# Priberam/Enhance-CB-Whisper

Measured on AMD Instinct MI355X. Metric: utterances/sec (30 s clips) + keywords/sec matched, Whisper-large-v3 LEF 10k kw, higher is better.
Workload: dtype bf16

## Files before the change

enhance-cb-whisper_amd/csrc/conv_igemm.hip:

```cpp
#include "cbw_common.h"
#include "cbw_kernels.h"
#include "conv_route.h"

#include <atomic>

thread_local const char* cbw_last_conv_kernel = "";

int cbw_num_cus() {
    static std::atomic<int> cache[16];
    int dev = 0, n = 0;
    (void)hipGetDevice(&dev);
    const bool slot = dev >= 0 && dev < 16;
    if (slot && (n = cache[dev].load(std::memory_order_relaxed)) > 0) return n;
    if (hipDeviceGetAttribute(&n, hipDeviceAttributeMultiprocessorCount, dev) != hipSuccess || n <= 0) n = 256;
    if (slot) cache[dev].store(n, std::memory_order_relaxed);
    return n;
}

namespace {

constexpr int BK = 64;
constexpr int EPI_LD = 68;
constexpr int EPI_BYTES = 4 * 64 * EPI_LD * 4;
template <int BM, int BN>
// ... 586 lines not shown
        const char* B = A + BIG_BM * 64;
        bf16x8 av[FM], bv[4];
#pragma unroll
        for (int j = 0; j < 4; ++j) {
            const int r = wn * 64 + j * 16 + fr;
            bv[j] = *(const bf16x8*)(B + r * 64 + ((fq ^ swz4(r)) * 16));
        }
#pragma unroll
        for (int i = 0; i < FH; ++i) {
            const int r = wm * (FM * 16) + i * 16 + fr;
            av[i] = *(const bf16x8*)(A + r * 64 + ((fq ^ swz4(r)) * 16));
        }
#pragma unroll
        for (int i = 0; i < FH; ++i) {
            __builtin_amdgcn_sched_barrier(0);
            __builtin_amdgcn_s_setprio(1);
#pragma unroll
            for (int j = 0; j < 4; ++j)
                acc[i][j] = __builtin_amdgcn_mfma_f32_16x16x32_bf16(bv[j], av[i], acc[i][j], 0, 0, 0);
            __builtin_amdgcn_s_setprio(0);
            __builtin_amdgcn_sched_barrier(0);
            const int r = wm * (FM * 16) + (i + FH) * 16 + fr;
            av[i + FH] = *(const bf16x8*)(A + r * 64 + ((fq ^ swz4(r)) * 16));
        }
        __builtin_amdgcn_sched_barrier(0);
        if (s + 3 < nsteps) issue_next();
        __builtin_amdgcn_sched_barrier(0);
        __builtin_amdgcn_s_setprio(1);
#pragma unroll
        for (int i = FH; i < FM; ++i)
#pragma unroll
            for (int j = 0; j < 4; ++j)
                acc[i][j] = __builtin_amdgcn_mfma_f32_16x16x32_bf16(bv[j], av[i], acc[i][j], 0, 0, 0);
        __builtin_amdgcn_s_setprio(0);
        asm volatile("" ::: "memory");
    }

    const bool relu = a.flags & CBW_EPI_RELU;
    const bool split3 = a.flags & CBW_EPI_SPLIT3;
#pragma unroll
    for (int j = 0; j < 4; ++j) {
        const int col = n0 + wn * 64 + j * 16 + fq * 4;
        const f32x4 bb = a.bias ? *(const f32x4*)(a.bias + col) : f32x4{0.f, 0.f, 0.f, 0.f};
#pragma unroll
        for (int i = 0; i < FM; ++i) {
            const int m = m0 + wm * (FM * 16) + i * 16 + fr;
            if (m >= a.M) continue;
            f32x4 v;
#pragma unroll
            for (int q = 0; q < 4; ++q) {
                v[q] = acc[i][j][q] + bb[q];
                if (relu) v[q] = fmaxf(v[q], 0.f);
            }
            bf16x4 o;
#pragma unroll
            for (int q = 0; q < 4; ++q) o[q] = f2bf(v[q]);
            bf16* yp = (bf16*)a.y + (int64_t)m * a.y_ld + col;
            *(bf16x4*)yp = o;
            if (split3) {
                bf16x4 lo;
#pragma unroll
                for (int q = 0; q < 4; ++q) lo[q] = f2bf(v[q] - bf2f(o[q]));
                *(bf16x4*)(yp + a.Cout) = lo;
                if (a.y32) *(f32x4*)(a.y32 + (int64_t)m * a.Cout + col) = v;
            }
        }
    }
}

template <int BN, int KH, int KW>
hipError_t launch_big(const ConvArgs& a, int nt, hipStream_t st) {
    constexpr int lds = BIG_NS * (BIG_BM + BN) * 64;
    hipLaunchKernelGGL((conv_igemm_big2<BN, KH, KW>), dim3(nt), dim3(512), lds, st, a);
    return hipGetLastError();
}

constexpr int P8_BM = 256, P8_BN = 256, P8_BK = 64;
CBW_DEV int p8_off(int r, int c) { return r * 128 + ((c ^ ((r >> 1) & 7)) << 4); }
template <int BN> struct P8Shape {
    static constexpr int BM = 65536 / BN;
    static constexpr int NA = BM / 128, NB = BN / 128;
    static constexpr int WCN = BN / 64;
    static constexpr int BUF = (BM + BN) * 128;
};
template <int N> CBW_DEV void vm_wait() {
    static_assert(N >= 0 && N <= 15, "vm_wait");
    asm volatile("s_waitcnt vmcnt(%0)" ::"n"(N) : "memory");
}

template <int KH, int KW, int BN = 256>
__global__ __launch_bounds__(512, 1) void conv_igemm_p8(ConvArgs a) {
    static_assert(KH * KW <= 32, "tap mask");
    using S = P8Shape<BN>;
    constexpr int BM = S::BM, NA = S::NA, NB = S::NB, WCN = S::WCN;
    extern __shared__ __attribute__((aligned(16))) char smem[];
    const int tid = threadIdx.x, lane = tid & 63, wid = tid >> 6;
    const int wr = (wid >> 2) * (4 / WCN) + (wid & 3) / WCN, wc = (wid & 3) % WCN;
    const int fr = lane & 15, fq = lane >> 4;
    const int nt_n = a.Cout / BN;
    const int nt_m = (a.M + BM - 1) / BM;
    const int bid = xcd_remap(blockIdx.x, nt_m * nt_n);
    const int tm = bid / nt_n, tn = bid % nt_n;
    const int m0 = tm * BM, n0 = tn * BN;
    const int cin2 = a.x2 ? a.Cin2 : 0;
    const int Ktot = KH * KW * a.Cin + cin2;
    const int csteps = a.Cin / P8_BK;
    const int nk1 = KH * KW * csteps;
    const int nk = nk1 + cin2 / P8_BK;
    const int HoWo = a.Ho * a.Wo;
    const int xld = a.x_ld ? a.x_ld : a.Cin;

    const int sub = lane >> 3, pch = lane & 7;
    const bf16* a_px[2][NA];
    const bf16* a2_px[2][NA];
    unsigned a_tm[2][NA];
    const bf16* wrow[2][NB];
    constexpr bool ROWS = KH * KW > 1;
    bool rowmap = false;
    int kh_lo = 0, kt_lo = 0, kt_hi = nk;
    if constexpr (ROWS) {
        rowmap = a.p8_g > 0;
        if (rowmap) {
            if (tid < BM) {
                int4 rec{-1, 0, 0, 0};
                if (m0 + tid < a.M) p8_row_pixel(m0 + tid, a.N, a.Ho, a.Wo, a.p8_g, rec.x, rec.y, rec.z, rec.w);
                ((int4*)smem)[tid] = rec;
            }
            __syncthreads();
            const int4 first = ((const int4*)smem)[0], last = ((const int4*)smem)[min(BM, a.M - m0) - 1];
            int kh_hi;
            p8_kh_range(__builtin_amdgcn_readfirstlane(first.y), __builtin_amdgcn_readfirstlane(last.y),
                        __builtin_amdgcn_readfirstlane(first.w) == __builtin_amdgcn_readfirstlane(last.w), a.H, a.sh,
                        a.ph, KH, kh_lo, kh_hi);
            kt_lo = kh_lo * KW * csteps;
            kt_hi = kh_hi * KW * csteps;
        }
    }
#pragma unroll
    for (int h = 0; h < 2; ++h)
#pragma unroll
        for (int g = 0; g < NA; ++g) {
            const int r = g * 128 + h * 64 + wid * 8 + sub;
            bool okm;
            int n, oh, ow;
            if (ROWS && rowmap) {
                const int4 rec = ((const int4*)smem)[r];
                okm = rec.x >= 0;
                n = okm ? rec.x : 0;
                oh = rec.y;
                ow = rec.z;
            } else {
                const int m = m0 + r;
                okm = m < a.M;
                const int mm = okm ? m : 0;
                n = mm / HoWo;
                const int rem = mm - n * HoWo;
                oh = rem / a.Wo;
                ow = rem - oh * a.Wo;
            }
            const int ih0 = oh * a.sh - a.ph, iw0 = ow * a.sw - a.pw;
            a2_px[h][g] = a.x2 ? (const bf16*)a.x2 + (((int64_t)n * a.H2 + oh * a.s2) * a.W2 + ow * a.s2) * cin2 +
                                     ((pch ^ ((r >> 1) & 7)) * 8)
                               : nullptr;
            unsigned tmask = 0;
#pragma unroll
            for (int kh = 0; kh < KH; ++kh)
#pragma unroll
                for (int kw = 0; kw < KW; ++kw) {
                    const int ih = ih0 + kh, iw = iw0 + kw;
                    if (okm && ih >= 0 && ih < a.H && iw >= 0 && iw < a.W) tmask |= 1u << (kh * KW + kw);
                }
            a_tm[h][g] = tmask;
            a_px[h][g] = (const bf16*)a.x + (int64_t)n * a.H * a.W * xld + ((int64_t)ih0 * a.W + iw0) * xld +
                         ((pch ^ ((r >> 1) & 7)) * 8);
        }
#pragma unroll
    for (int h = 0; h < 2; ++h)
#pragma unroll
        for (int g = 0; g < NB; ++g) {
            const int rb = h * (BN / 2) + g * 64 + wid * 8 + sub;
            const int rs = (rb & ~31) | (((rb & 15) >> 2) << 3) | (((rb >> 4) & 1) << 2) | (rb & 3);
            wrow[h][g] = (const bf16*)a.w + (int64_t)(n0 + rs) * Ktot + ((pch ^ ((rb >> 1) & 7)) * 8);
        }
    int nx_cs = 0, nx_tap = 0, nx_kh = 0, nx_kw = 0;
    if constexpr (ROWS) {
        nx_kh = kh_lo;
        nx_tap = nx_kh * KW;
        if (rowmap) __syncthreads();
    }
    int nx_off = nx_kh * a.W * xld + fold_c(0, a.xfold);
    auto advance = [&]() {
        if (++nx_cs == csteps) {
            nx_cs = 0;
            ++nx_tap;
            if (++nx_kw == KW) { nx_kw = 0; ++nx_kh; }
        }
        nx_off = (nx_kh * a.W + nx_kw) * xld + fold_c(nx_cs * P8_BK, a.xfold);
    };
    auto issue = [&](int kt, int which) {
        char* A = smem + (kt & 1) * S::BUF;
        if (which == 0 || which == 3) {
            const int h = which == 3;
            if (kt >= nk1) {
                const int c0 = (kt - nk1) * P8_BK;
#pragma unroll
                for (int g = 0; g < NA; ++g) {
                    const void* src = (a_tm[h][g] & 1u) ? (const void*)(a2_px[h][g] + c0) : a.zero;
                    __builtin_amdgcn_global_load_lds(src, (void*)(A + (g * 128 + h * 64 + wid * 8) * 128), 16, 0, 0);
                }
                return;
            }
            const int tap = nx_tap;
            const int toff = nx_off;
#pragma unroll
            for (int g = 0; g < NA; ++g) {
                const void* src = ((a_tm[h][g] >> tap) & 1u) ? (const void*)(a_px[h][g] + toff) : a.zero;
                __builtin_amdgcn_global_load_lds(src, (void*)(A + (g * 128 + h * 64 + wid * 8) * 128), 16, 0, 0);
            }
        } else {
            const int h = which - 1;
            char* B = A + BM * 128;
#pragma unroll
            for (int g = 0; g < NB; ++g)
                __builtin_amdgcn_global_load_lds((const void*)(wrow[h][g] + (int64_t)kt * P8_BK),
                                                 (void*)(B + (h * (BN / 2) + g * 64 + wid * 8) * 128), 16, 0, 0);
        }
    };

    f32x4 acc[8][4];
#pragma unroll
    for (int i = 0; i < 8; ++i)
#pragma unroll
        for (int j = 0; j < 4; ++j) acc[i][j] = f32x4{0.f, 0.f, 0.f, 0.f};
    bf16x8 av[4][2], bv[2][2];

#pragma unroll
    for (int w = 0; w < 4; ++w) issue(kt_lo, w);
    advance();
    asm volatile("s_waitcnt vmcnt(0)" ::: "memory");
    __builtin_amdgcn_s_barrier();
    if (wid >= 4) __builtin_amdgcn_s_barrier();
    for (int kt = kt_lo; kt < kt_hi; ++kt) {
        const char* A = smem + (kt & 1) * S::BUF;
        const char* B = A + BM * 128;
        const bool more = kt + 1 < kt_hi;
#pragma unroll
        for (int q = 0; q < 4; ++q) {
            const int mi = q >> 1, ni = (q == 1 || q == 2) ? 1 : 0;
            __builtin_amdgcn_sched_barrier(0);
            if (more) {
                issue(kt + 1, q);
                if (q == 3) advance();
                if (q == 0) vm_wait<2 * NA>();
                else if (q == 2) vm_wait<2 * NB>();
                else vm_wait<NA + NB>();
            } else if (q == 0) {
                vm_wait<NA>();
            } else {
                vm_wait<0>();
            }
            if (q == 0 || q == 2) {
#pragma unroll
                for (int i = 0; i < 4; ++i)
#pragma unroll
                    for (int ks = 0; ks < 2; ++ks)
                        av[i][ks] = *(const bf16x8*)(A + p8_off(wr * 128 + mi * 64 + i * 16 + fr, ks * 4 + fq));
            }
            if (q != 2) {
#pragma unroll
                for (int j = 0; j < 2; ++j)
#pragma unroll
                    for (int ks = 0; ks < 2; ++ks)
                        bv[j][ks] = *(const bf16x8*)(B + p8_off(ni * (BN / 2) + wc * 32 + j * 16 + fr, ks * 4 + fq));
            }
            __builtin_amdgcn_sched_barrier(0);
            __builtin_amdgcn_s_barrier();
            __builtin_amdgcn_s_setprio(1);
#pragma unroll
            for (int ks = 0; ks < 2; ++ks)
#pragma unroll
                for (int i = 0; i < 4; ++i)
#pragma unroll
                    for (int j = 0; j < 2; ++j)
                        acc[mi * 4 + i][ni * 2 + j] =
                            __builtin_amdgcn_mfma_f32_16x16x32_bf16(bv[j][ks], av[i][ks], acc[mi * 4 + i][ni * 2 + j], 0, 0, 0);
            __builtin_amdgcn_s_setprio(0);
            __builtin_amdgcn_sched_barrier(0);
            __builtin_amdgcn_s_barrier();
        }
    }
    if (wid < 4) __builtin_amdgcn_s_barrier();

    const int flags = a.flags;
    const bool relu = flags & CBW_EPI_RELU;
    const bool has_res = a.res != nullptr;
    const bool res_split = flags & CBW_EPI_RES_SPLIT, res_f32 = flags & CBW_EPI_RES_F32;
    if constexpr (ROWS) {
        if (rowmap) {
            if (tid < BM) {
                int n, oh, ow, grp, m = -1;
                if (m0 + tid < a.M) {
                    p8_row_pixel(m0 + tid, a.N, a.Ho, a.Wo, a.p8_g, n, oh, ow, grp);
                    m = (n * a.Ho + oh) * a.Wo + ow;
                }
                ((int*)smem)[tid] = m;
            }
            __syncthreads();
        }
    }
    auto row_m = [&](int f) {
        if (ROWS && rowmap) return ((const int*)smem)[wr * 128 + f * 16 + fr];
        return m0 + wr * 128 + f * 16 + fr;
    };
#pragma unroll
    for (int ni = 0; ni < 2; ++ni) {
        const int col = n0 + ni * (BN / 2) + wc * 32 + fq * 8;
        f32x4 bb[2] = {f32x4{0.f, 0.f, 0.f, 0.f}, f32x4{0.f, 0.f, 0.f, 0.f}};
        if (a.bias) {
            bb[0] = *(const f32x4*)(a.bias + col);
            bb[1] = *(const f32x4*)(a.bias + col + 4);
        }
        uint4 rw0[8], rw1[8];
        if (has_res) {
#pragma unroll
            for (int f = 0; f < 8; ++f) {
                const int mc = (ROWS && rowmap) ? max(row_m(f), 0) : min(row_m(f), a.M - 1);
                if (res_f32) {
                    const float* rp = (const float*)a.res + (int64_t)mc * a.res_ld + col;
                    rw0[f] = *(const uint4*)rp;
                    rw1[f] = *(const uint4*)(rp + 4);
                } else {
                    const bf16* rp = (const bf16*)a.res + (int64_t)mc * a.res_ld + col;
                    rw0[f] = *(const uint4*)rp;
                    if (res_split) rw1[f] = *(const uint4*)(rp + a.Cout);
                }
            }
        }
#pragma unroll
        for (int f = 0; f < 8; ++f) {
            const int m = row_m(f);
            if ((ROWS && rowmap) ? m < 0 : m >= a.M) continue;
            float v[8];
#pragma unroll
            for (int j = 0; j < 2; ++j)
#pragma unroll
                for (int q = 0; q < 4; ++q) v[4 * j + q] = acc[f][ni * 2 + j][q] + bb[j][q];
            if (has_res) {
                float rv[8];
                if (res_split) {
                    const bf16x8 hi = __builtin_bit_cast(bf16x8, rw0[f]), lo = __builtin_bit_cast(bf16x8, rw1[f]);
#pragma unroll
                    for (int q = 0; q < 8; ++q) rv[q] = bf2f(hi[q]) + bf2f(lo[q]);
                } else if (res_f32) {
                    const f32x4 r0 = __builtin_bit_cast(f32x4, rw0[f]), r1 = __builtin_bit_cast(f32x4, rw1[f]);
#pragma unroll
                    for (int q = 0; q < 4; ++q) { rv[q] = r0[q]; rv[q + 4] = r1[q]; }
                } else {
                    const bf16x8 r = __builtin_bit_cast(bf16x8, rw0[f]);
#pragma unroll
                    for (int q = 0; q < 8; ++q) rv[q] = bf2f(r[q]);
                }
#pragma unroll
                for (int q = 0; q < 8; ++q) v[q] += rv[q];
            }
            if (relu)
#pragma unroll
                for (int q = 0; q < 8; ++q) v[q] = fmaxf(v[q], 0.f);
            store_out8(a, flags, m, col, v);
        }
    }
}

static_assert(BK == CONV_BK && P8_BK == CONV_BK && P8_BM == conv_p8_bm(P8_BN) && P8Shape<128>::BM == conv_p8_bm(128) &&
                  BIG_BM == CONV_BIG_BM && BIG_BK == CONV_BIG_BK,
              "conv_route.h decides for these tiles");

template <int KH, int KW, int BN>
hipError_t launch_p8(const ConvArgs& a0, const ConvRoute& r, hipStream_t st) {
    using S = P8Shape<BN>;
    ConvArgs a = a0;
    a.p8_g = r.p8_g;
    if (BN != 256) {
        static const hipError_t attr = hipFuncSetAttribute((const void*)conv_igemm_p8<KH, KW, BN>,
                                                           hipFuncAttributeMaxDynamicSharedMemorySize, 2 * S::BUF);
        if (attr != hipSuccess) return attr;
    }
    hipLaunchKernelGGL((conv_igemm_p8<KH, KW, BN>), dim3(r.tiles), dim3(512), 2 * S::BUF, st, a);
    return hipGetLastError();
}

template <int BM, int BN, int KH, int KW>
hipError_t launch_persist(const ConvArgs& a, int ntiles, hipStream_t st) {
    const int G = std::min(ntiles, 2 * cbw_num_cus());
    constexpr int lds = 2 * (BM + BN) * 128 + 4 * 8 * EPI_LD * 4;
    hipLaunchKernelGGL((conv_igemm_persist<BM, BN, KH, KW>), dim3(G), dim3(256), lds, st, a, ntiles);
    return hipGetLastError();
}

template <int BM, int BN, int KH, int KW>
hipError_t launch_t(const ConvArgs& a, int nt, hipStream_t st) {
    constexpr int lds = lds_bytes<BM, BN>();
    hipLaunchKernelGGL((conv_igemm_kernel<BM, BN, KH, KW>), dim3(nt), dim3(256), lds, st, a);
    return hipGetLastError();
}

template <int KH, int KW>
hipError_t launch_k(const ConvArgs& a, const ConvRoute& r, hipStream_t st) {
    switch (r.kernel) {
        case ConvKernel::Stream: return cbw_conv_stream(a, r, st);
        case ConvKernel::Ring: return cbw_conv_ring(a, r, st);
        case ConvKernel::P8:
            return r.BN == 256 ? launch_p8<KH, KW, 256>(a, r, st) : launch_p8<KH, KW, 128>(a, r, st);
        case ConvKernel::Big2: return launch_big<256, KH, KW>(a, r.tiles, st);
        case ConvKernel::Persist: return launch_persist<128, 128, KH, KW>(a, r.tiles, st);
        case ConvKernel::Tile:
            return r.BN == 128 ? launch_t<128, 128, KH, KW>(a, r.tiles, st) : launch_t<256, 64, KH, KW>(a, r.tiles, st);
        default: return hipErrorInvalidValue;
    }
}

}

namespace {
__global__ __launch_bounds__(256) void splitk_epilogue_kernel(ConvArgs a, int S) {
    const int64_t n4 = (int64_t)a.M * a.Cout / 4;
    for (int64_t e = blockIdx.x * (int64_t)blockDim.x + threadIdx.x; e < n4; e += (int64_t)gridDim.x * blockDim.x) {
        const int64_t i = e * 4;
        const int m = (int)(i / a.Cout), col = (int)(i - (int64_t)m * a.Cout);
        f32x4 v = *(const f32x4*)(a.partial + i);
        for (int z = 1; z < S; ++z) v += *(const f32x4*)(a.partial + (int64_t)z * a.M * a.Cout + i);
        if (a.bias) v += *(const f32x4*)(a.bias + col);
        float rv[4] = {0.f, 0.f, 0.f, 0.f};
        const bool has_res = a.res != nullptr;
        if (has_res) {
            if (a.flags & CBW_EPI_RES_F32) {
                const f32x4 r = *(const f32x4*)((const float*)a.res + (int64_t)m * a.res_ld + col);
#pragma unroll
                for (int q = 0; q < 4; ++q) rv[q] = r[q];
            } else {
                const bf16x4 r = *(const bf16x4*)((const bf16*)a.res + (int64_t)m * a.res_ld + col);
#pragma unroll
                for (int q = 0; q < 4; ++q) rv[q] = bf2f(r[q]);
            }
            if (!(a.flags & CBW_EPI_RES_AFTER_ACT))
#pragma unroll
                for (int q = 0; q < 4; ++q) v[q] += rv[q];
        }
#pragma unroll
        for (int q = 0; q < 4; ++q) {
            if (a.flags & CBW_EPI_RELU) v[q] = fmaxf(v[q], 0.f);
            else if (a.flags & CBW_EPI_GELU) v[q] = gelu_erf(v[q]);
            if (has_res && (a.flags & CBW_EPI_RES_AFTER_ACT)) v[q] += rv[q];
        }
        if (a.flags & CBW_EPI_OUT_F32) {
            *(f32x4*)((float*)a.y + (int64_t)m * a.y_ld + col) = v;
        } else {
            bf16x4 o;
#pragma unroll
            for (int q = 0; q < 4; ++q) o[q] = f2bf(v[q]);
            *(bf16x4*)((bf16*)a.y + (int64_t)m * a.y_ld + col) = o;
        }
    }
}
}

int cbw_conv_splitk_factor(const ConvArgs& a) { return conv_splitk_factor(a, cbw_num_cus()); }

hipError_t cbw_conv_igemm_splitk(const ConvArgs& a0, int ksplit, float* partial, hipStream_t st) {
    if (ksplit <= 1 || partial == nullptr) return cbw_conv_igemm(a0, st);
    if (a0.KH != 1 || a0.KW != 1 || a0.x2 != nullptr || a0.Cout % 128 || a0.Cin % BK || a0.Cout % 4 ||
        a0.y_ld % 4 || (a0.res && a0.res_ld % 4) || ksplit > a0.Cin / BK)
        return hipErrorInvalidValue;
    ConvArgs a = a0;
    a.ksplit = ksplit;
    a.partial = partial;
    const int nt = ((a.M + 127) / 128) * (a.Cout / 128);
    constexpr int lds = lds_bytes<128, 128>();
    cbw_last_conv_kernel = "conv_igemm_kernel<128, 128, 1, 1> + splitk_epilogue_kernel";
    hipLaunchKernelGGL((conv_igemm_kernel<128, 128, 1, 1>), dim3(nt, ksplit), dim3(256), lds, st, a);
    const int64_t n4 = (int64_t)a.M * a.Cout / 4;
    const int grid = (int)std::min<int64_t>((n4 + 255) / 256, 4 * cbw_num_cus());
    hipLaunchKernelGGL(splitk_epilogue_kernel, dim3(grid), dim3(256), 0, st, a, ksplit);
    return hipGetLastError();
}

hipError_t cbw_conv_igemm(const ConvArgs& a, hipStream_t st) {
    const ConvRoute r = conv_route(a, cbw_num_cus(), conv_knobs_from_env());
    if (r.kernel == ConvKernel::Invalid) return hipErrorInvalidValue;
    cbw_last_conv_kernel = r.name;
    if (a.KW == 1) return launch_k<1, 1>(a, r, st);
    if (a.KH == 3) return launch_k<3, 3>(a, r, st);
    return launch_k<1, 3>(a, r, st);
}
```

enhance-cb-whisper_amd/csrc/conv_route.h:

```cpp
#pragma once
#include <stdint.h>
#include <stdlib.h>

#include "conv_args.h"
#include "p8_rowmap.h"

enum class ConvKernel { Invalid, Stream, Chain, Ring, P8, Big2, Persist, Tile };

struct ConvStreamVariant {
    int ks, waves, rd, pfd, pn;
};

struct ConvRoute {
    ConvKernel kernel = ConvKernel::Invalid;
    int BM = 0, BN = 0;
    int tiles = 0;
    int p8_g = 0;
    ConvStreamVariant stream = {};
    const char* name = "";
};

struct ConvKnobs {
    int conv_p8 = 1;
    int p8_x2 = 1;
    int p8_tier = 1;
    int p8_n128 = 1;
    int p8_rowskip = 1;
    int p8_rowgroup = 0;
    int conv_stream = 1;
    int cs_k512 = 1;
    int cs_prefetch = -1;
    int cs_chain = 1;
};

inline ConvKnobs conv_knobs_from_env() {
    ConvKnobs k;
    const auto read = [](const char* name, int& v) {
        if (const char* e = getenv(name)) v = atoi(e);
    };
    read("CBW_CONV_P8", k.conv_p8);
    read("CBW_P8_X2", k.p8_x2);
    read("CBW_P8_TIER", k.p8_tier);
    read("CBW_P8_N128", k.p8_n128);
    read("CBW_P8_ROWSKIP", k.p8_rowskip);
    read("CBW_P8_ROWGROUP", k.p8_rowgroup);
    read("CBW_CONV_STREAM", k.conv_stream);
    read("CBW_CS_K512", k.cs_k512);
    read("CBW_CS_PREFETCH", k.cs_prefetch);
    read("CBW_CS_CHAIN", k.cs_chain);
    return k;
}

constexpr int CONV_BK = 64;
constexpr int CONV_BIG_BM = 256, CONV_BIG_BK = 32;
constexpr int CONV_RING_BM = 256, CONV_RING_BN = 128, CONV_RING_BK = 64, CONV_RING_MAXC = 2048;
constexpr int CONV_CS_WBYTES = 131072, CONV_CS_MAXSLICE = 1024;
constexpr int CONV_CC_K = 128, CONV_CC_N = 512, CONV_CC_R = 128;
constexpr int conv_p8_bm(int BN) { return 65536 / BN; }

inline int conv_ktot(const ConvArgs& a) { return a.KH * a.KW * a.Cin + (a.x2 ? a.Cin2 : 0); }
inline int conv_tiles(const ConvArgs& a, int BM, int BN) { return ((a.M + BM - 1) / BM) * (a.Cout / BN); }

#define CBW_NAME_BY_TAPS(a, pre, post) \
    ((a).KH == 3 ? pre "3, 3" post : (a).KW == 3 ? pre "1, 3" post : pre "1, 1" post)

inline int slice_channels(int cout, int ktot) {
    for (int nsl = 1; nsl <= cout / 128; ++nsl) {
        if (cout % nsl) continue;
        const int sn = cout / nsl;
        if (sn % 128 == 0 && sn <= CONV_CS_MAXSLICE && (int64_t)sn * ktot * 2 <= CONV_CS_WBYTES) return sn;
    }
    return 0;
}

inline bool conv_stream_supported(const ConvArgs& a, const ConvKnobs& k) {
    const int ktot = a.Cin + (a.x2 ? a.Cin2 : 0);
    if (a.KH != 1 || a.KW != 1 || a.sh != 1 || a.sw != 1 || a.ph != 0 || a.pw != 0) return false;
    if (ktot != 128 && ktot != 256 && ktot != 384 && !(ktot == 512 && k.cs_k512)) return false;
    if (a.Cin % 32 || (a.x2 && a.Cin2 % 32)) return false;
    if (a.flags & ~CBW_EPI_RELU) return false;
    if (a.res && a.res_ld % 4) return false;
    if (a.y_ld % 4 || a.M <= 0) return false;
    const int64_t lim = 0x7ffffff0LL - 4096;
    if ((int64_t)a.M * a.y_ld * 2 >= lim || (int64_t)a.M * a.Cin * 2 >= lim) return false;
    if (a.res && (int64_t)a.M * a.res_ld * 2 >= lim) return false;
    if (a.x2 && (int64_t)a.N * a.H2 * a.W2 * a.Cin2 * 2 >= lim) return false;
    return slice_channels(a.Cout, ktot) > 0;
}

inline bool conv_stream_wanted(const ConvArgs& a, const ConvKnobs& k) {
    return k.conv_stream != 0 && conv_stream_supported(a, k);
}

inline ConvRoute conv_stream_route(const ConvArgs& a, const ConvKnobs& k) {
    ConvRoute r;
    if (!conv_stream_supported(a, k)) return r;
    const int ktot = a.Cin + (a.x2 ? a.Cin2 : 0);
    const bool pn = k.cs_prefetch >= 0 ? k.cs_prefetch != 0 : (ktot == 128 || (ktot == 256 && !a.res));
    r.kernel = ConvKernel::Stream;
#define CBW_CS_VARIANT(KS, WAVES, RD, PFD, PN) \
    (r.stream = ConvStreamVariant{KS, WAVES, RD, PFD, PN},  \
     r.name = "conv_stream_kernel<" #KS ", " #WAVES ", " #RD ", " #PFD ", " #PN ">")
    switch (ktot) {
        case 128: pn ? CBW_CS_VARIANT(4, 8, 2, 2, 1) : CBW_CS_VARIANT(4, 12, 2, 2, 0); break;
        case 256: pn ? CBW_CS_VARIANT(8, 8, 1, 2, 1) : CBW_CS_VARIANT(8, 12, 1, 2, 0); break;
        case 512: CBW_CS_VARIANT(16, 8, 2, 1, 0); break;
        default: CBW_CS_VARIANT(12, 8, 2, 2, 0); break;
    }
#undef CBW_CS_VARIANT
    return r;
}

inline bool conv_chain_supported(const ConvArgs& a, int red_cout, const ConvKnobs& k) {
    if (!conv_stream_supported(a, k) || a.x2 || a.Cin != CONV_CC_K || a.Cout != CONV_CC_N || red_cout != CONV_CC_R)
        return false;
    if (!a.res || a.flags != CBW_EPI_RELU || a.y_ld != CONV_CC_N) return false;
    return slice_channels(a.Cout, a.Cin) == a.Cout;
}

inline ConvRoute conv_chain_route(const ConvArgs& a, int red_cout, const ConvKnobs& k) {
    ConvRoute r;
    if (!conv_chain_supported(a, red_cout, k)) return r;
    r.kernel = ConvKernel::Chain;
    r.name = "conv_stream_chain_kernel<4, 2, 4>";
    return r;
}

inline ConvRoute conv_junction_route(const ConvArgs& a, const ConvArgs& r, const ConvKnobs& k) {
    if (!k.cs_chain || r.Cin != a.Cout || r.flags != CBW_EPI_RELU) return {};
    if (!conv_stream_wanted(a, k) || !conv_stream_wanted(r, k)) return {};
    return conv_chain_route(a, r.Cout, k);
}

inline bool conv_ring_supported(const ConvArgs& a) {
    if (a.Cout % CONV_RING_BN || a.Cout > CONV_RING_MAXC || a.Cin % CONV_RING_BK || a.M <= 0) return false;
    if (a.flags & ~CBW_EPI_RELU) return false;
    if (a.res) return false;
    if (a.y_ld % 4 || (int64_t)a.M * a.y_ld * 2 >= 0x7fffffffLL) return false;
    if (a.x2 && (a.KH * a.KW != 1 || a.Cin2 % CONV_RING_BK)) return false;
    return (a.KH == 1 && a.KW == 1) || (a.KH == 3 && a.KW == 3);
}

inline bool ring_wanted(const ConvArgs& a) {
    return conv_ring_supported(a) && a.KH * a.KW == 1 && a.res == nullptr && conv_ktot(a) <= 768;
}

inline ConvRoute conv_ring_route(const ConvArgs& a) {
    ConvRoute r;
    if (!conv_ring_supported(a)) return r;
    r.kernel = ConvKernel::Ring;
    r.BM = CONV_RING_BM, r.BN = CONV_RING_BN;
    r.tiles = conv_tiles(a, r.BM, r.BN);
    r.name = a.KH == 1 ? "conv_ring_kernel<1, 1>" : "conv_ring_kernel<3, 3>";
    return r;
}

inline bool p8_shape(const ConvArgs& a, const ConvKnobs& k, int BN) {
    return k.conv_p8 == 1 && a.Cout % 256 == BN % 256 && a.Cin % CONV_BK == 0 && a.xfold % CONV_BK == 0;
}
inline bool p8_epilogue(const ConvArgs& a) { return !(a.flags & (CBW_EPI_GELU | CBW_EPI_RES_AFTER_ACT)); }

inline int p8_rowgroup(const ConvArgs& a, const ConvKnobs& k, int BM) {
    if (a.KH * a.KW == 1 || k.p8_rowskip == 0 || a.N <= 0 || (int64_t)a.N * a.Ho * a.Wo != a.M) return 0;
    const int G = k.p8_rowgroup > 0 ? k.p8_rowgroup : p8_default_rowgroup(a.Wo, BM);
    return G < a.N ? G : a.N;
}

inline ConvRoute conv_route(const ConvArgs& a, int ncus, const ConvKnobs& k) {
    const int taps = a.KH * a.KW;
    const auto tile_route = [&](ConvKernel kernel, int BM, int BN, const char* name) {
        ConvRoute r;
        r.kernel = kernel;
        r.BM = BM, r.BN = BN;
        r.tiles = conv_tiles(a, BM, BN);
        r.name = name;
        return r;
    };
    const auto p8_route = [&](int BN) {
        ConvRoute r = tile_route(ConvKernel::P8, conv_p8_bm(BN), BN,
                                 BN == 256 ? CBW_NAME_BY_TAPS(a, "conv_igemm_p8<", ", 256>")
                                           : CBW_NAME_BY_TAPS(a, "conv_igemm_p8<", ", 128>"));
        r.p8_g = p8_rowgroup(a, k, r.BM);
        return r;
    };
    const auto big2_route = [&] {
        return tile_route(ConvKernel::Big2, CONV_BIG_BM, 256, CBW_NAME_BY_TAPS(a, "conv_igemm_big2<256, ", ">"));
    };
    if (!((a.KH == 1 && a.KW == 1) || (a.KH == 3 && a.KW == 3) || (a.KH == 1 && a.KW == 3))) return {};
    if (a.x2 != nullptr && (taps != 1 || a.Cin2 % CONV_BK)) return {};
    const int64_t xld = a.x_ld ? a.x_ld : a.Cin;
    if (((int64_t)(a.KH - 1) * a.W + (a.KW - 1)) * xld + a.Cin + (a.x2 ? a.Cin2 : 0) > INT32_MAX) return {};

    const int ktot = taps * a.Cin;
    const bool tile_only = a.xfold || (a.x_ld && a.x_ld != a.Cin) || (a.flags & (CBW_EPI_SPLIT3 | CBW_EPI_RES_SPLIT));
    const bool plain = a.res == nullptr && !(a.flags & (CBW_EPI_OUT_F32 | CBW_EPI_GELU | CBW_EPI_RES_SPLIT));
    const bool p8_256 = p8_shape(a, k, 256);
    const bool fills = conv_tiles(a, 256, 256) >= ncus;

    const bool x2_fit = a.x2 && plain && p8_256 && ktot + a.Cin2 >= 512 && !a.xfold && !a.x_ld && fills;
    if (x2_fit && k.p8_x2 >= 2) return p8_route(256);
    if (!tile_only && taps == 1 && conv_stream_wanted(a, k)) return conv_stream_route(a, k);
    if (x2_fit && k.p8_x2 >= 1) return p8_route(256);
    if (k.p8_tier && (a.flags & (CBW_EPI_SPLIT3 | CBW_EPI_OUT_F32)) && a.xfold && a.x2 == nullptr && p8_256 &&
        p8_epilogue(a) && ktot >= 512 && (fills || (ktot >= 4096 && 2 * conv_tiles(a, 256, 256) >= ncus)))
        return p8_route(256);
    if (!tile_only && ring_wanted(a)) return conv_ring_route(a);
    const bool big_ok = plain && a.x2 == nullptr && a.Cin % CONV_BIG_BK == 0 && a.xfold % CONV_BIG_BK == 0 && ktot >= 256;
    if (big_ok && fills && a.Cout % 256 == 0) return p8_256 ? p8_route(256) : big2_route();
    if (big_ok && k.p8_n128 && p8_shape(a, k, 128) && ktot >= 512 && conv_tiles(a, 512, 128) >= ncus)
        return p8_route(128);
    if (a.Cin % CONV_BK || a.Cout % 64) return big_ok && a.Cout % 256 == 0 ? big2_route() : ConvRoute{};
    if (a.Cout % 128 == 0) {
        const bool short_k = taps * (a.Cin / CONV_BK) == 1;
        if (a.x2 != nullptr || short_k || a.res != nullptr)
            return tile_route(ConvKernel::Persist, 128, 128, CBW_NAME_BY_TAPS(a, "conv_igemm_persist<128, 128, ", ">"));
        return tile_route(ConvKernel::Tile, 128, 128, CBW_NAME_BY_TAPS(a, "conv_igemm_kernel<128, 128, ", ">"));
    }
    if (a.x2 != nullptr) return {};
    return tile_route(ConvKernel::Tile, 256, 64, CBW_NAME_BY_TAPS(a, "conv_igemm_kernel<256, 64, ", ">"));
}

inline int conv_splitk_factor(const ConvArgs& a, int ncus) {
    if (a.KH != 1 || a.KW != 1 || a.x2 != nullptr || a.Cout % 128 || a.Cin % CONV_BK) return 1;
    const int tiles = conv_tiles(a, 128, 128), slots = 2 * ncus, nsteps = a.Cin / CONV_BK;
    int S = 1;
    while (S < 8 && tiles * (S * 2) <= slots && nsteps / (S * 2) >= 4) S *= 2;
    return S;
}
```

Before: 6.286.

## Make p8 conv kernel persistent, prefetching next tile during epilogue

The p8 implicit-GEMM conv kernel now launches at most one block per CU (BN=256) and walks tiles in a grid-stride loop. It sets up and issues the first K-step loads for the next tile before running the epilogue of the current one, so global loads overlap with output stores. Row records are double-buffered in extra LDS, and the epilogue processes rows in smaller batches to limit register pressure. Optional cycle-stamp instrumentation and a conv_p8=2 force-route knob are added; tile scheduling and tail balance may change.

New measurement: 6.313, median of 6. About the same (+0.4%).

```diff
diff --git a/enhance-cb-whisper_amd/csrc/conv_igemm.hip b/enhance-cb-whisper_amd/csrc/conv_igemm.hip
--- a/enhance-cb-whisper_amd/csrc/conv_igemm.hip
+++ b/enhance-cb-whisper_amd/csrc/conv_igemm.hip
@@ -692,7 +692,25 @@
     static constexpr int NA = BM / 128, NB = BN / 128;
     static constexpr int WCN = BN / 64;
     static constexpr int BUF = (BM + BN) * 128;
+    static constexpr bool WALK = 2 * BUF + 2 * BM * 16 <= 160 * 1024;
+    static constexpr int LDS = WALK ? 2 * BUF + 2 * BM * 16 : 2 * BUF;
 };
+static_assert(P8Shape<256>::WALK && !P8Shape<128>::WALK, "conv_route.h: p8 walks tiles at BN = 256 only");
+
+#ifdef CBW_P8_STAMPS
+constexpr int P8_STAMPS = 10;
+__device__ unsigned long long* p8_stamp_buf = nullptr;
+__device__ int p8_stamp_cap = 0;
+#define P8_STAMP_V(tile, slot, value)                                                              \
+    do {                                                                                           \
+        if (threadIdx.x == 0 && p8_stamp_buf != nullptr && (tile) < p8_stamp_cap)                   \
+            p8_stamp_buf[(int64_t)(tile) * P8_STAMPS + (slot)] = (unsigned long long)(value);      \
+    } while (0)
+#define P8_STAMP(tile, slot) P8_STAMP_V(tile, slot, __builtin_readcyclecounter())
+#else
+#define P8_STAMP_V(tile, slot, value) do {} while (0)
+#define P8_STAMP(tile, slot) do {} while (0)
+#endif
 template <int N> CBW_DEV void vm_wait() {
     static_assert(N >= 0 && N <= 15, "vm_wait");
     asm volatile("s_waitcnt vmcnt(%0)" ::"n"(N) : "memory");
@@ -709,10 +727,9 @@
     const int fr = lane & 15, fq = lane >> 4;
     const int nt_n = a.Cout / BN;
     const int nt_m = (a.M + BM - 1) / BM;
-    const int bid = xcd_remap(blockIdx.x, nt_m * nt_n);
-    const int tm = bid / nt_n, tn = bid % nt_n;
-    const int m0 = tm * BM, n0 = tn * BN;
-    const int cin2 = a.x2 ? a.Cin2 : 0;
+    const int ntiles = nt_m * nt_n;
+    int m0 = 0, n0 = 0;
+    const int cin2 = (KH * KW == 1 && a.x2) ? a.Cin2 : 0;
     const int Ktot = KH * KW * a.Cin + cin2;
     const int csteps = a.Cin / P8_BK;
     const int nk1 = KH * KW * csteps;
@@ -724,81 +741,85 @@
     const bf16* a_px[2][NA];
     const bf16* a2_px[2][NA];
     unsigned a_tm[2][NA];
-    const bf16* wrow[2][NB];
-    constexpr bool ROWS = KH * KW > 1;
-    bool rowmap = false;
-    int kh_lo = 0, kt_lo = 0, kt_hi = nk;
-    if constexpr (ROWS) {
-        rowmap = a.p8_g > 0;
-        if (rowmap) {
-            if (tid < BM) {
-                int4 rec{-1, 0, 0, 0};
-                if (m0 + tid < a.M) p8_row_pixel(m0 + tid, a.N, a.Ho, a.Wo, a.p8_g, rec.x, rec.y, rec.z, rec.w);
-                ((int4*)smem)[tid] = rec;
-            }
-            __syncthreads();
-            const int4 first = ((const int4*)smem)[0], last = ((const int4*)smem)[min(BM, a.M - m0) - 1];
-            int kh_hi;
-            p8_kh_range(__builtin_amdgcn_readfirstlane(first.y), __builtin_amdgcn_readfirstlane(last.y),
-                        __builtin_amdgcn_readfirstlane(first.w) == __builtin_amdgcn_readfirstlane(last.w), a.H, a.sh,
-                        a.ph, KH, kh_lo, kh_hi);
-            kt_lo = kh_lo * KW * csteps;
-            kt_hi = kh_hi * KW * csteps;
-        }
-    }
-#pragma unroll
-    for (int h = 0; h < 2; ++h)
-#pragma unroll
-        for (int g = 0; g < NA; ++g) {
-            const int r = g * 128 + h * 64 + wid * 8 + sub;
-            bool okm;
-            int n, oh, ow;
-            if (ROWS && rowmap) {
-                const int4 rec = ((const int4*)smem)[r];
-                okm = rec.x >= 0;
-                n = okm ? rec.x : 0;
-                oh = rec.y;
-                ow = rec.z;
-            } else {
-                const int m = m0 + r;
-                okm = m < a.M;
-                const int mm = okm ? m : 0;
-                n = mm / HoWo;
-                const int rem = mm - n * HoWo;
-                oh = rem / a.Wo;
-                ow = rem - oh * a.Wo;
-            }
-            const int ih0 = oh * a.sh - a.ph, iw0 = ow * a.sw - a.pw;
-            a2_px[h][g] = a.x2 ? (const bf16*)a.x2 + (((int64_t)n * a.H2 + oh * a.s2) * a.W2 + ow * a.s2) * cin2 +
-                                     ((pch ^ ((r >> 1) & 7)) * 8)
-                               : nullptr;
-            unsigned tmask = 0;
-#pragma unroll
-            for (int kh = 0; kh < KH; ++kh)
-#pragma unroll
-                for (int kw = 0; kw < KW; ++kw) {
-                    const int ih = ih0 + kh, iw = iw0 + kw;
-                    if (okm && ih >= 0 && ih < a.H && iw >= 0 && iw < a.W) tmask |= 1u << (kh * KW + kw);
+    const bf16* wrow;
+    constexpr bool ROWS = KH * KW > 1, WALK = S::WALK;
+    const bool rowmap = ROWS && a.p8_g > 0;
+    auto recs = [&](int p) { return (int4*)(smem + (WALK ? 2 * S::BUF + p * BM * 16 : 0)); };
+    auto decode_rows = [&](int p) {
+        if (tid < BM) {
+            int4 rec{-1, 0, 0, 0};
+            if (m0 + tid < a.M) p8_row_pixel(m0 + tid, a.N, a.Ho, a.Wo, a.p8_g, rec.x, rec.y, rec.z, rec.w);
+            recs(p)[tid] = rec;
+        }
+        __syncthreads();
+    };
+    int kt_lo = 0, kt_hi = nk;
+    int nx_cs = 0, nx_tap = 0, nx_kh = 0, nx_kw = 0, nx_off = 0;
+    auto setup = [&](int vt, int p) {
+        const int bid = xcd_remap(vt, ntiles);
+        const int tm = bid / nt_n, tn = bid % nt_n;
+        m0 = tm * BM, n0 = tn * BN;
+        int kh_lo = 0;
+        kt_lo = 0, kt_hi = nk;
+        if constexpr (ROWS) {
+            if (rowmap) {
+                decode_rows(p);
+                const int4 first = recs(p)[0], last = recs(p)[min(BM, a.M - m0) - 1];
+                int kh_hi;
+                p8_kh_range(__builtin_amdgcn_readfirstlane(first.y), __builtin_amdgcn_readfirstlane(last.y),
+                            __builtin_amdgcn_readfirstlane(first.w) == __builtin_amdgcn_readfirstlane(last.w), a.H,
+                            a.sh, a.ph, KH, kh_lo, kh_hi);
+                kt_lo = kh_lo * KW * csteps;
+                kt_hi = kh_hi * KW * csteps;
+            }
+        }
+#pragma unroll
+        for (int h = 0; h < 2; ++h)
+#pragma unroll
+            for (int g = 0; g < NA; ++g) {
+                const int r = g * 128 + h * 64 + wid * 8 + sub;
+                bool okm;
+                int n, oh, ow;
+                if (ROWS && rowmap) {
+                    const int4 rec = recs(p)[r];
+                    okm = rec.x >= 0;
+                    n = okm ? rec.x : 0;
+                    oh = rec.y;
+                    ow = rec.z;
+                } else {
+                    const int m = m0 + r;
+                    okm = m < a.M;
+                    const int mm = okm ? m : 0;
+                    n = mm / HoWo;
+                    const int rem = mm - n * HoWo;
+                    oh = rem / a.Wo;
+                    ow = rem - oh * a.Wo;
                 }
-            a_tm[h][g] = tmask;
-            a_px[h][g] = (const bf16*)a.x + (int64_t)n * a.H * a.W * xld + ((int64_t)ih0 * a.W + iw0) * xld +
-                         ((pch ^ ((r >> 1) & 7)) * 8);
-        }
-#pragma unroll
-    for (int h = 0; h < 2; ++h)
-#pragma unroll
-        for (int g = 0; g < NB; ++g) {
-            const int rb = h * (BN / 2) + g * 64 + wid * 8 + sub;
+                const int ih0 = oh * a.sh - a.ph, iw0 = ow * a.sw - a.pw;
+                a2_px[h][g] = !ROWS && a.x2 ? (const bf16*)a.x2 + (((int64_t)n * a.H2 + oh * a.s2) * a.W2 + ow * a.s2) * cin2 +
+                                         ((pch ^ ((r >> 1) & 7)) * 8)
+                                   : nullptr;
+                unsigned tmask = 0;
+#pragma unroll
+                for (int kh = 0; kh < KH; ++kh)
+#pragma unroll
+                    for (int kw = 0; kw < KW; ++kw) {
+                        const int ih = ih0 + kh, iw = iw0 + kw;
+                        if (okm && ih >= 0 && ih < a.H && iw >= 0 && iw < a.W) tmask |= 1u << (kh * KW + kw);
+                    }
+                a_tm[h][g] = tmask;
+                a_px[h][g] = (const bf16*)a.x + (int64_t)n * a.H * a.W * xld + ((int64_t)ih0 * a.W + iw0) * xld +
+                             ((pch ^ ((r >> 1) & 7)) * 8);
+            }
+        {
+            const int rb = wid * 8 + sub;
             const int rs = (rb & ~31) | (((rb & 15) >> 2) << 3) | (((rb >> 4) & 1) << 2) | (rb & 3);
-            wrow[h][g] = (const bf16*)a.w + (int64_t)(n0 + rs) * Ktot + ((pch ^ ((rb >> 1) & 7)) * 8);
-        }
-    int nx_cs = 0, nx_tap = 0, nx_kh = 0, nx_kw = 0;
-    if constexpr (ROWS) {
-        nx_kh = kh_lo;
-        nx_tap = nx_kh * KW;
-        if (rowmap) __syncthreads();
-    }
-    int nx_off = nx_kh * a.W * xld + fold_c(0, a.xfold);
+            wrow = (const bf16*)a.w + (int64_t)(n0 + rs) * Ktot + ((pch ^ ((rb >> 1) & 7)) * 8);
+        }
+        nx_cs = 0, nx_kw = 0, nx_kh = kh_lo, nx_tap = kh_lo * KW;
+        if (ROWS && !WALK && rowmap) __syncthreads();
+        nx_off = nx_kh * a.W * xld + fold_c(0, a.xfold);
+    };
     auto advance = [&]() {
         if (++nx_cs == csteps) {
             nx_cs = 0;
@@ -811,7 +832,7 @@
         char* A = smem + (kt & 1) * S::BUF;
         if (which == 0 || which == 3) {
             const int h = which == 3;
-            if (kt >= nk1) {
+            if (!ROWS && kt >= nk1) {
                 const int c0 = (kt - nk1) * P8_BK;
 #pragma unroll
                 for (int g = 0; g < NA; ++g) {
@@ -832,152 +853,196 @@
             char* B = A + BM * 128;
 #pragma unroll
             for (int g = 0; g < NB; ++g)
-                __builtin_amdgcn_global_load_lds((const void*)(wrow[h][g] + (int64_t)kt * P8_BK),
+                __builtin_amdgcn_global_load_lds((const void*)(wrow + ((int64_t)(h * (BN / 2) + g * 64) * Ktot + kt * P8_BK)),
                                                  (void*)(B + (h * (BN / 2) + g * 64 + wid * 8) * 128), 16, 0, 0);
         }
     };
 
+    auto first_fill = [&]() {
+#pragma unroll
+        for (int w = 0; w < 4; ++w) issue(kt_lo, w);
+        advance();
+    };
+
     f32x4 acc[8][4];
-#pragma unroll
-    for (int i = 0; i < 8; ++i)
-#pragma unroll
-        for (int j = 0; j < 4; ++j) acc[i][j] = f32x4{0.f, 0.f, 0.f, 0.f};
     bf16x8 av[4][2], bv[2][2];
-
-#pragma unroll
-    for (int w = 0; w < 4; ++w) issue(kt_lo, w);
-    advance();
-    asm volatile("s_waitcnt vmcnt(0)" ::: "memory");
-    __builtin_amdgcn_s_barrier();
-    if (wid >= 4) __builtin_amdgcn_s_barrier();
-    for (int kt = kt_lo; kt < kt_hi; ++kt) {
-        const char* A = smem + (kt & 1) * S::BUF;
-        const char* B = A + BM * 128;
-        const bool more = kt + 1 < kt_hi;
-#pragma unroll
-        for (int q = 0; q < 4; ++q) {
-            const int mi = q >> 1, ni = (q == 1 || q == 2) ? 1 : 0;
-            __builtin_amdgcn_sched_barrier(0);
-            if (more) {
-                issue(kt + 1, q);
-                if (q == 3) advance();
-                if (q == 0) vm_wait<2 * NA>();
-                else if (q == 2) vm_wait<2 * NB>();
-                else vm_wait<NA + NB>();
-            } else if (q == 0) {
-                vm_wait<NA>();
-            } else {
-                vm_wait<0>();
-            }
-            if (q == 0 || q == 2) {
-#pragma unroll
-                for (int i = 0; i < 4; ++i)
-#pragma unroll
-                    for (int ks = 0; ks < 2; ++ks)
-                        av[i][ks] = *(const bf16x8*)(A + p8_off(wr * 128 + mi * 64 + i * 16 + fr, ks * 4 + fq));
-            }
-            if (q != 2) {
-#pragma unroll
-                for (int j = 0; j < 2; ++j)
-#pragma unroll
-                    for (int ks = 0; ks < 2; ++ks)
-                        bv[j][ks] = *(const bf16x8*)(B + p8_off(ni * (BN / 2) + wc * 32 + j * 16 + fr, ks * 4 + fq));
-            }
-            __builtin_amdgcn_sched_barrier(0);
-            __builtin_amdgcn_s_barrier();
-            __builtin_amdgcn_s_setprio(1);
-#pragma unroll
-            for (int ks = 0; ks < 2; ++ks)
-#pragma unroll
-                for (int i = 0; i < 4; ++i)
-#pragma unroll
-                    for (int j = 0; j < 2; ++j)
-                        acc[mi * 4 + i][ni * 2 + j] =
-                            __builtin_amdgcn_mfma_f32_16x16x32_bf16(bv[j][ks], av[i][ks], acc[mi * 4 + i][ni * 2 + j], 0, 0, 0);
-            __builtin_amdgcn_s_setprio(0);
-            __builtin_amdgcn_sched_barrier(0);
-            __builtin_amdgcn_s_barrier();
-        }
-    }
-    if (wid < 4) __builtin_amdgcn_s_barrier();
-
     const int flags = a.flags;
     const bool relu = flags & CBW_EPI_RELU;
     const bool has_res = a.res != nullptr;
     const bool res_split = flags & CBW_EPI_RES_SPLIT, res_f32 = flags & CBW_EPI_RES_F32;
-    if constexpr (ROWS) {
-        if (rowmap) {
-            if (tid < BM) {
-                int n, oh, ow, grp, m = -1;
-                if (m0 + tid < a.M) {
-                    p8_row_pixel(m0 + tid, a.N, a.Ho, a.Wo, a.p8_g, n, oh, ow, grp);
-                    m = (n * a.Ho + oh) * a.Wo + ow;
+
+    f32x4 bb[2][2];
+
+    auto k_loop = [&](int vt) {
+#pragma unroll
+        for (int i = 0; i < 8; ++i)
+#pragma unroll
+            for (int j = 0; j < 4; ++j) acc[i][j] = f32x4{0.f, 0.f, 0.f, 0.f};
+        asm volatile("s_waitcnt vmcnt(0)" ::: "memory");
+        __builtin_amdgcn_s_barrier();
+        P8_STAMP(vt, 2);
+        if (wid >= 4) __builtin_amdgcn_s_barrier();
+        for (int kt = kt_lo; kt < kt_hi; ++kt) {
+            const char* A = smem + (kt & 1) * S::BUF;
+            const char* B = A + BM * 128;
+            const bool more = kt + 1 < kt_hi;
+#pragma unroll
+            for (int q = 0; q < 4; ++q) {
+                const int mi = q >> 1, ni = (q == 1 || q == 2) ? 1 : 0;
+                __builtin_amdgcn_sched_barrier(0);
+                if (more) {
+                    issue(kt + 1, q);
+                    if (q == 3) advance();
+                    if (q == 0) vm_wait<2 * NA>();
+                    else if (q == 2) vm_wait<2 * NB>();
+                    else vm_wait<NA + NB>();
+                } else if (q == 0) {
+                    vm_wait<NA>();
+                } else {
+                    vm_wait<0>();
                 }
-                ((int*)smem)[tid] = m;
-            }
-            __syncthreads();
-        }
-    }
-    auto row_m = [&](int f) {
-        if (ROWS && rowmap) return ((const int*)smem)[wr * 128 + f * 16 + fr];
-        return m0 + wr * 128 + f * 16 + fr;
+                if (q == 0 || q == 2) {
+#pragma unroll
+                    for (int i = 0; i < 4; ++i)
+#pragma unroll
+                        for (int ks = 0; ks < 2; ++ks)
+                            av[i][ks] = *(const bf16x8*)(A + p8_off(wr * 128 + mi * 64 + i * 16 + fr, ks * 4 + fq));
+                }
+                if (q != 2) {
+#pragma unroll
+                    for (int j = 0; j < 2; ++j)
+#pragma unroll
+                        for (int ks = 0; ks < 2; ++ks)
+                            bv[j][ks] =
+                                *(const bf16x8*)(B + p8_off(ni * (BN / 2) + wc * 32 + j * 16 + fr, ks * 4 + fq));
+                }
+                __builtin_amdgcn_sched_barrier(0);
+                __builtin_amdgcn_s_barrier();
+                __builtin_amdgcn_s_setprio(1);
+#pragma unroll
+                for (int ks = 0; ks < 2; ++ks)
+#pragma unroll
+                    for (int i = 0; i < 4; ++i)
+#pragma unroll
+                        for (int j = 0; j < 2; ++j)
+                            acc[mi * 4 + i][ni * 2 + j] = __builtin_amdgcn_mfma_f32_16x16x32_bf16(
+                                bv[j][ks], av[i][ks], acc[mi * 4 + i][ni * 2 + j], 0, 0, 0);
+                __builtin_amdgcn_s_setprio(0);
+                __builtin_amdgcn_sched_barrier(0);
+                __builtin_amdgcn_s_barrier();
+            }
+        }
+        if (wid < 4) __builtin_amdgcn_s_barrier();
     };
-#pragma unroll
-    for (int ni = 0; ni < 2; ++ni) {
-        const int col = n0 + ni * (BN / 2) + wc * 32 + fq * 8;
-        f32x4 bb[2] = {f32x4{0.f, 0.f, 0.f, 0.f}, f32x4{0.f, 0.f, 0.f, 0.f}};
-        if (a.bias) {
-            bb[0] = *(const f32x4*)(a.bias + col);
-            bb[1] = *(const f32x4*)(a.bias + col + 4);
-        }
-        uint4 rw0[8], rw1[8];
-        if (has_res) {
-#pragma unroll
-            for (int f = 0; f < 8; ++f) {
-                const int mc = (ROWS && rowmap) ? max(row_m(f), 0) : min(row_m(f), a.M - 1);
-                if (res_f32) {
-                    const float* rp = (const float*)a.res + (int64_t)mc * a.res_ld + col;
-                    rw0[f] = *(const uint4*)rp;
-                    rw1[f] = *(const uint4*)(rp + 4);
-                } else {
-                    const bf16* rp = (const bf16*)a.res + (int64_t)mc * a.res_ld + col;
-                    rw0[f] = *(const uint4*)rp;
-                    if (res_split) rw1[f] = *(const uint4*)(rp + a.Cout);
+
+    auto epilogue = [&](int vt, int em0, int en0, int ep) {
+        constexpr int RB = WALK ? 4 : 8;
+        auto row_m = [&](int f) {
+            if (ROWS && rowmap) {
+                const int4 rec = recs(ep)[wr * 128 + f * 16 + fr];
+                return rec.x < 0 ? -1 : (rec.x * a.Ho + rec.y) * a.Wo + rec.z;
+            }
+            return em0 + wr * 128 + f * 16 + fr;
+        };
+#pragma unroll
+        for (int ni = 0; ni < 2; ++ni) {
+            const int col = en0 + ni * (BN / 2) + wc * 32 + fq * 8;
+#pragma unroll
+            for (int f0 = 0; f0 < 8; f0 += RB) {
+                uint4 rw0[RB], rw1[RB];
+                if (has_res) {
+#pragma unroll
+                    for (int f = f0; f < f0 + RB; ++f) {
+                        const int mc = (ROWS && rowmap) ? max(row_m(f), 0) : min(row_m(f), a.M - 1);
+                        if (res_f32) {
+                            const float* rp = (const float*)a.res + (int64_t)mc * a.res_ld + col;
+                            rw0[f - f0] = *(const uint4*)rp;
+                            rw1[f - f0] = *(const uint4*)(rp + 4);
+                        } else {
+                            const bf16* rp = (const bf16*)a.res + (int64_t)mc * a.res_ld + col;
+                            rw0[f - f0] = *(const uint4*)rp;
+                            if (res_split) rw1[f - f0] = *(const uint4*)(rp + a.Cout);
+                        }
+                    }
                 }
-            }
-        }
-#pragma unroll
-        for (int f = 0; f < 8; ++f) {
-            const int m = row_m(f);
-            if ((ROWS && rowmap) ? m < 0 : m >= a.M) continue;
-            float v[8];
-#pragma unroll
-            for (int j = 0; j < 2; ++j)
-#pragma unroll
-                for (int q = 0; q < 4; ++q) v[4 * j + q] = acc[f][ni * 2 + j][q] + bb[j][q];
-            if (has_res) {
-                float rv[8];
-                if (res_split) {
-                    const bf16x8 hi = __builtin_bit_cast(bf16x8, rw0[f]), lo = __builtin_bit_cast(bf16x8, rw1[f]);
-#pragma unroll
-                    for (int q = 0; q < 8; ++q) rv[q] = bf2f(hi[q]) + bf2f(lo[q]);
-                } else if (res_f32) {
-                    const f32x4 r0 = __builtin_bit_cast(f32x4, rw0[f]), r1 = __builtin_bit_cast(f32x4, rw1[f]);
-#pragma unroll
-                    for (int q = 0; q < 4; ++q) { rv[q] = r0[q]; rv[q + 4] = r1[q]; }
-                } else {
-                    const bf16x8 r = __builtin_bit_cast(bf16x8, rw0[f]);
-#pragma unroll
-                    for (int q = 0; q < 8; ++q) rv[q] = bf2f(r[q]);
+#ifdef CBW_P8_STAMPS
+                if (ni == 0 && f0 == 0) {
+                    vm_wait<0>();
+                    P8_STAMP(vt, 4);
                 }
-#pragma unroll
-                for (int q = 0; q < 8; ++q) v[q] += rv[q];
-            }
-            if (relu)
-#pragma unroll
-                for (int q = 0; q < 8; ++q) v[q] = fmaxf(v[q], 0.f);
-            store_out8(a, flags, m, col, v);
-        }
+#endif
+#pragma unroll
+                for (int f = f0; f < f0 + RB; ++f) {
+                    const int m = row_m(f);
+                    if ((ROWS && rowmap) ? m < 0 : m >= a.M) continue;
+                    float v[8];
+#pragma unroll
+                    for (int j = 0; j < 2; ++j)
+#pragma unroll
+                        for (int q = 0; q < 4; ++q) v[4 * j + q] = acc[f][ni * 2 + j][q] + bb[ni][j][q];
+                    if (has_res) {
+                        float rv[8];
+                        if (res_split) {
+                            const bf16x8 hi = __builtin_bit_cast(bf16x8, rw0[f - f0]), lo = __builtin_bit_cast(bf16x8, rw1[f - f0]);
+#pragma unroll
+                            for (int q = 0; q < 8; ++q) rv[q] = bf2f(hi[q]) + bf2f(lo[q]);
+                        } else if (res_f32) {
+                            const f32x4 r0 = __builtin_bit_cast(f32x4, rw0[f - f0]), r1 = __builtin_bit_cast(f32x4, rw1[f - f0]);
+#pragma unroll
+                            for (int q = 0; q < 4; ++q) { rv[q] = r0[q]; rv[q + 4] = r1[q]; }
+                        } else {
+                            const bf16x8 r = __builtin_bit_cast(bf16x8, rw0[f - f0]);
+#pragma unroll
+                            for (int q = 0; q < 8; ++q) rv[q] = bf2f(r[q]);
+                        }
+#pragma unroll
+                        for (int q = 0; q < 8; ++q) v[q] += rv[q];
+                    }
+                    if (relu)
+#pragma unroll
+                        for (int q = 0; q < 8; ++q) v[q] = fmaxf(v[q], 0.f);
+                    store_out8(a, flags, m, col, v);
+                }
+            }
+        }
+    };
+
+    int vt = blockIdx.x, par = 0;
+    P8_STAMP(vt, 0);
+    P8_STAMP_V(vt, 7, wall_clock64());
+    P8_STAMP_V(vt, 9, blockIdx.x);
+    setup(vt, par);
+    P8_STAMP(vt, 1);
+    first_fill();
+    for (;;) {
+        k_loop(vt);
+        P8_STAMP(vt, 3);
+        const int em0 = m0, en0 = n0;
+#pragma unroll
+        for (int h = 0; h < 2; ++h) {
+            const float* bp = a.bias + en0 + h * (BN / 2) + wc * 32 + fq * 8;
+            bb[h][0] = a.bias ? *(const f32x4*)bp : f32x4{0.f, 0.f, 0.f, 0.f};
+            bb[h][1] = a.bias ? *(const f32x4*)(bp + 4) : f32x4{0.f, 0.f, 0.f, 0.f};
+        }
+        const int nvt = vt + gridDim.x;
+        const bool walk = WALK && nvt < ntiles;
+        if (walk) {
+            setup(nvt, par ^ 1);
+            first_fill();
+            __builtin_amdgcn_sched_barrier(0);
+        } else if (ROWS && !WALK && rowmap) {
+            decode_rows(par);
+        }
+        P8_STAMP(vt, 6);
+        epilogue(vt, em0, en0, par);
+        P8_STAMP(vt, 5);
+        P8_STAMP_V(vt, 8, wall_clock64());
+        if (!walk) break;
+        vt = nvt;
+        par ^= 1;
+        P8_STAMP(vt, 0);
+        P8_STAMP_V(vt, 7, wall_clock64());
+        P8_STAMP_V(vt, 9, blockIdx.x);
     }
 }
 
@@ -990,12 +1055,11 @@
     using S = P8Shape<BN>;
     ConvArgs a = a0;
     a.p8_g = r.p8_g;
-    if (BN != 256) {
-        static const hipError_t attr = hipFuncSetAttribute((const void*)conv_igemm_p8<KH, KW, BN>,
-                                                           hipFuncAttributeMaxDynamicSharedMemorySize, 2 * S::BUF);
-        if (attr != hipSuccess) return attr;
-    }
-    hipLaunchKernelGGL((conv_igemm_p8<KH, KW, BN>), dim3(r.tiles), dim3(512), 2 * S::BUF, st, a);
+    static const hipError_t attr = hipFuncSetAttribute((const void*)conv_igemm_p8<KH, KW, BN>,
+                                                       hipFuncAttributeMaxDynamicSharedMemorySize, S::LDS);
+    if (attr != hipSuccess) return attr;
+    if (r.grid < 1 || r.grid > r.tiles || (r.grid < r.tiles && !S::WALK)) return hipErrorInvalidValue;
+    hipLaunchKernelGGL((conv_igemm_p8<KH, KW, BN>), dim3(r.grid), dim3(512), S::LDS, st, a);
     return hipGetLastError();
 }
 
@@ -1094,6 +1158,14 @@
     return hipGetLastError();
 }
 
+#ifdef CBW_P8_STAMPS
+extern "C" int cbw_p8_set_stamps(void* buf, int cap) {
+    if (hipMemcpyToSymbol(HIP_SYMBOL(p8_stamp_buf), &buf, sizeof(buf)) != hipSuccess) return -2;
+    if (hipMemcpyToSymbol(HIP_SYMBOL(p8_stamp_cap), &cap, sizeof(cap)) != hipSuccess) return -2;
+    return P8_STAMPS;
+}
+#endif
+
 hipError_t cbw_conv_igemm(const ConvArgs& a, hipStream_t st) {
     const ConvRoute r = conv_route(a, cbw_num_cus(), conv_knobs_from_env());
     if (r.kernel == ConvKernel::Invalid) return hipErrorInvalidValue;
diff --git a/enhance-cb-whisper_amd/csrc/conv_route.h b/enhance-cb-whisper_amd/csrc/conv_route.h
--- a/enhance-cb-whisper_amd/csrc/conv_route.h
+++ b/enhance-cb-whisper_amd/csrc/conv_route.h
@@ -16,6 +16,7 @@
     int BM = 0, BN = 0;
     int tiles = 0;
     int p8_g = 0;
+    int grid = 0;
     ConvStreamVariant stream = {};
     const char* name = "";
 };
@@ -27,6 +28,8 @@
     int p8_n128 = 1;
     int p8_rowskip = 1;
     int p8_rowgroup = 0;
+    int p8_persist = 1;
+    int p8_grid = 0;
     int conv_stream = 1;
     int cs_k512 = 1;
     int cs_prefetch = -1;
@@ -44,6 +47,8 @@
     read("CBW_P8_N128", k.p8_n128);
     read("CBW_P8_ROWSKIP", k.p8_rowskip);
     read("CBW_P8_ROWGROUP", k.p8_rowgroup);
+    read("CBW_P8_PERSIST", k.p8_persist);
+    read("CBW_P8_GRID", k.p8_grid);
     read("CBW_CONV_STREAM", k.conv_stream);
     read("CBW_CS_K512", k.cs_k512);
     read("CBW_CS_PREFETCH", k.cs_prefetch);
@@ -156,7 +161,7 @@
 }
 
 inline bool p8_shape(const ConvArgs& a, const ConvKnobs& k, int BN) {
-    return k.conv_p8 == 1 && a.Cout % 256 == BN % 256 && a.Cin % CONV_BK == 0 && a.xfold % CONV_BK == 0;
+    return k.conv_p8 >= 1 && a.Cout % 256 == BN % 256 && a.Cin % CONV_BK == 0 && a.xfold % CONV_BK == 0;
 }
 inline bool p8_epilogue(const ConvArgs& a) { return !(a.flags & (CBW_EPI_GELU | CBW_EPI_RES_AFTER_ACT)); }
 
@@ -164,6 +169,12 @@
     if (a.KH * a.KW == 1 || k.p8_rowskip == 0 || a.N <= 0 || (int64_t)a.N * a.Ho * a.Wo != a.M) return 0;
     const int G = k.p8_rowgroup > 0 ? k.p8_rowgroup : p8_default_rowgroup(a.Wo, BM);
     return G < a.N ? G : a.N;
+}
+
+inline int p8_grid(int tiles, int BN, int ncus, const ConvKnobs& k) {
+    if (BN != 256 || k.p8_persist == 0) return tiles;
+    const int cap = k.p8_grid > 0 && k.p8_grid < ncus ? k.p8_grid : ncus;
+    return tiles < cap ? tiles : cap;
 }
 
 inline ConvRoute conv_route(const ConvArgs& a, int ncus, const ConvKnobs& k) {
@@ -181,6 +192,7 @@
                                  BN == 256 ? CBW_NAME_BY_TAPS(a, "conv_igemm_p8<", ", 256>")
                                            : CBW_NAME_BY_TAPS(a, "conv_igemm_p8<", ", 128>"));
         r.p8_g = p8_rowgroup(a, k, r.BM);
+        r.grid = p8_grid(r.tiles, BN, ncus, k);
         return r;
     };
     const auto big2_route = [&] {
@@ -196,6 +208,7 @@
     const bool plain = a.res == nullptr && !(a.flags & (CBW_EPI_OUT_F32 | CBW_EPI_GELU | CBW_EPI_RES_SPLIT));
     const bool p8_256 = p8_shape(a, k, 256);
     const bool fills = conv_tiles(a, 256, 256) >= ncus;
+    if (k.conv_p8 == 2 && p8_256 && p8_epilogue(a) && (a.x2 == nullptr || (!a.xfold && !a.x_ld))) return p8_route(256);
 
     const bool x2_fit = a.x2 && plain && p8_256 && ktot + a.Cin2 >= 512 && !a.xfold && !a.x_ld && fills;
     if (x2_fit && k.p8_x2 >= 2) return p8_route(256);
```
